# luokn/ms-gat

Measured on AMD Instinct MI355X. Metric: MS-GAT fwd+bwd samples/sec (B×T node-updates/s), PEMSD7 N=883 T=12, higher is better.
Workload: dtype f32

## Files before the change

### ms_gat_amd/csrc/scores.hip

```cpp
#include "common.hpp"

namespace msgat {

constexpr int kRowBlock = 256;

__global__ __launch_bounds__(kBlock) void k_edge_grad(const float* __restrict__ dEp, int nchunks,
                                                      const float* __restrict__ E, const int* __restrict__ epos,
                                                      int stride, float* __restrict__ gE, int nnz) {
  const int g = blockIdx.y;
  const int e = blockIdx.x * kBlock + threadIdx.x;
  if (e >= nnz) return;
  const float* p = dEp + (size_t)g * nchunks * stride + (epos != nullptr ? epos[e] : e);
  float a0 = 0.f, a1 = 0.f, a2 = 0.f, a3 = 0.f;
  int k = 0;
  for (; k + 4 <= nchunks; k += 4) {
    a0 += p[(size_t)(k + 0) * stride];
    a1 += p[(size_t)(k + 1) * stride];
    a2 += p[(size_t)(k + 2) * stride];
    a3 += p[(size_t)(k + 3) * stride];
  }
  for (; k < nchunks; ++k) a0 += p[(size_t)k * stride];
  gE[(size_t)g * nnz + e] = E[(size_t)g * nnz + e] * ((a0 + a1) + (a2 + a3));
}

__global__ __launch_bounds__(kBlock) void k_edge_grad_csc(const float* __restrict__ dEp, int nchunks,
                                                          const float* __restrict__ Ec, const int* __restrict__ cperm,
                                                          float* __restrict__ gE, int nnz) {
  const int g = blockIdx.y;
  const int k = blockIdx.x * kBlock + threadIdx.x;
  if (k >= nnz) return;
  const float* p = dEp + (size_t)g * nchunks * nnz + k;
  float a[8] = {0.f, 0.f, 0.f, 0.f, 0.f, 0.f, 0.f, 0.f};
  const float ec = Ec[(size_t)g * nnz + k];
  const int dst = cperm[k];
  int c = 0;
  for (; c + 8 <= nchunks; c += 8) {
#pragma unroll
    for (int i = 0; i < 8; ++i) a[i] += p[(size_t)(c + i) * nnz];
  }
  for (; c < nchunks; ++c) a[0] += p[(size_t)c * nnz];
  gE[(size_t)g * nnz + dst] = ec * (((a[0] + a[1]) + (a[2] + a[3])) + ((a[4] + a[5]) + (a[6] + a[7])));
}

__global__ __launch_bounds__(kBlock) void k_edge_grad_x(const float* __restrict__ dEp, int nchunks,
                                                        const float* __restrict__ E, const int* __restrict__ epos,
                                                        int stride, float* __restrict__ gE, int nnz,
                                                        const float* __restrict__ dEx) {
  const int g = blockIdx.y;
  const int e = blockIdx.x * kBlock + threadIdx.x;
  if (e >= nnz) return;
  const float* p = dEp + (size_t)g * nchunks * stride + (epos != nullptr ? epos[e] : e);
  float a0 = 0.f, a1 = 0.f, a2 = 0.f, a3 = 0.f;
  int k = 0;
  for (; k + 4 <= nchunks; k += 4) {
    a0 += p[(size_t)(k + 0) * stride];
    a1 += p[(size_t)(k + 1) * stride];
    a2 += p[(size_t)(k + 2) * stride];
    a3 += p[(size_t)(k + 3) * stride];
  }
  for (; k < nchunks; ++k) a0 += p[(size_t)k * stride];
  const size_t i = (size_t)g * nnz + e;
  gE[i] = E[i] * (((a0 + a1) + (a2 + a3)) + dEx[i]);
}

__global__ __launch_bounds__(kBlock) void k_edge_grad_csc_x(const float* __restrict__ dEp, int nchunks,
                                                            const float* __restrict__ Ec, const int* __restrict__ cperm,
                                                            float* __restrict__ gE, int nnz, const float* __restrict__ dEx) {
  const int g = blockIdx.y;
  const int k = blockIdx.x * kBlock + threadIdx.x;
  if (k >= nnz) return;
  const float* p = dEp + (size_t)g * nchunks * nnz + k;
  float a[8] = {0.f, 0.f, 0.f, 0.f, 0.f, 0.f, 0.f, 0.f};
  const float ec = Ec[(size_t)g * nnz + k];
  const int dst = cperm[k];
  int c = 0;
  for (; c + 8 <= nchunks; c += 8) {
#pragma unroll
    for (int i = 0; i < 8; ++i) a[i] += p[(size_t)(c + i) * nnz];
  }
  for (; c < nchunks; ++c) a[0] += p[(size_t)c * nnz];
  const size_t i = (size_t)g * nnz + dst;
  gE[i] = ec * ((((a[0] + a[1]) + (a[2] + a[3])) + ((a[4] + a[5]) + (a[6] + a[7]))) + dEx[i]);
}


template <int T, int DC>
__global__ __launch_bounds__(kRowBlock) void k_bwd_rows(
    const int* __restrict__ rowptr, const int* __restrict__ col, const float* __restrict__ E,
    const float* __restrict__ u, const float* __restrict__ dv,
    const float* __restrict__ q, const float* __restrict__ pq, const float* __restrict__ Wg,
    float* gE, float* __restrict__ delta, float* __restrict__ dkW, float* __restrict__ dq,
    float* __restrict__ dwg_part, int Bg, int N, int nnz, int nblk) {
  constexpr int T4 = T / 4;
  constexpr int DCa = DC < 0 ? -DC : DC;
  constexpr int DCn = DCa > 0 ? DCa : 1;
  __shared__ float qs[kRowBlock * T];
  __shared__ float ds[kRowBlock * T];
  const int g = blockIdx.y;
  const int r = g / Bg;
  const int n = blockIdx.x * kRowBlock + threadIdx.x;
  const bool valid = n < N;
  const int nc = valid ? n : 0;
  const float* qg = q + (size_t)g * N * T;
  float d = 0.f;
  float dk[T], pr[T];
#pragma unroll
  for (int t4 = 0; t4 < T4; ++t4) {
    const float4 v = reinterpret_cast<const float4*>(pq + ((size_t)g * N + nc) * T)[t4];
    pr[4 * t4 + 0] = v.x; pr[4 * t4 + 1] = v.y; pr[4 * t4 + 2] = v.z; pr[4 * t4 + 3] = v.w;
    dk[4 * t4 + 0] = 0.f; dk[4 * t4 + 1] = 0.f; dk[4 * t4 + 2] = 0.f; dk[4 * t4 + 3] = 0.f;
  }
  float4 dvr[DCn][T4];
  if (DCa > 0) {
#pragma unroll
    for (int c = 0; c < DCn; ++c)
#pragma unroll
      for (int t4 = 0; t4 < T4; ++t4)
        dvr[c][t4] = reinterpret_cast<const float4*>(dv + (((size_t)g * DCa + c) * N + nc) * T)[t4];
  }
  auto edge_grad = [&](int e, int ce) -> float {
    float dE;
    if (DCa > 0) {
      dE = 0.f;
#pragma unroll
      for (int c = 0; c < DCn; ++c) {
        const float4* um = reinterpret_cast<const float4*>(u + (((size_t)g * DCa + c) * N + ce) * T);
#pragma unroll
        for (int t4 = 0; t4 < T4; ++t4) dE = f4dot(dvr[c][t4], um[t4], dE);
      }
    } else {
      return gE[(size_t)g * nnz + e];
    }
    if constexpr (DC < 0) dE += gE[(size_t)g * nnz + e];
    return E[(size_t)g * nnz + e] * dE;
  };
  const int e0 = valid ? rowptr[n] : 0;
  const int e1 = valid ? rowptr[n + 1] : 0;
  for (int e = e0; e < e1; e += 4) {
    int ee[4], cc[4];
#pragma unroll
    for (int i = 0; i < 4; ++i) {
      ee[i] = min(e + i, e1 - 1);
      cc[i] = col[ee[i]];
    }
    float gg[4];
#pragma unroll
    for (int i = 0; i < 4; ++i) {
      const float raw = edge_grad(ee[i], cc[i]);
      gg[i] = (e + i < e1) ? raw : 0.f;
    }
    if (DCa > 0) {
#pragma unroll
      for (int i = 0; i < 4; ++i)
        if (e + i < e1) gE[(size_t)g * nnz + ee[i]] = gg[i];
    }
    float4 qv[4][T4];
#pragma unroll
    for (int i = 0; i < 4; ++i)
#pragma unroll
      for (int t4 = 0; t4 < T4; ++t4) qv[i][t4] = reinterpret_cast<const float4*>(qg + (size_t)cc[i] * T)[t4];
#pragma unroll
    for (int i = 0; i < 4; ++i) {
      d += gg[i];
#pragma unroll
      for (int t4 = 0; t4 < T4; ++t4) {
        dk[4 * t4 + 0] = fmaf(gg[i], qv[i][t4].x - pr[4 * t4 + 0], dk[4 * t4 + 0]);
        dk[4 * t4 + 1] = fmaf(gg[i], qv[i][t4].y - pr[4 * t4 + 1], dk[4 * t4 + 1]);
        dk[4 * t4 + 2] = fmaf(gg[i], qv[i][t4].z - pr[4 * t4 + 2], dk[4 * t4 + 2]);
        dk[4 * t4 + 3] = fmaf(gg[i], qv[i][t4].w - pr[4 * t4 + 3], dk[4 * t4 + 3]);
      }
    }
  }
  if (valid) {
    float4* dkdst = reinterpret_cast<float4*>(dkW + ((size_t)g * N + n) * T);
#pragma unroll
    for (int t4 = 0; t4 < T4; ++t4) dkdst[t4] = make_float4(dk[4 * t4], dk[4 * t4 + 1], dk[4 * t4 + 2], dk[4 * t4 + 3]);
    delta[(size_t)g * N + n] = d;
    const float* wg = Wg + (size_t)r * T * T;
    float out[T];
#pragma unroll
    for (int t = 0; t < T; ++t) {
      float a = 0.f;
#pragma unroll
      for (int s = 0; s < T; ++s) a = fmaf(dk[s], wg[t * T + s], a);
      out[t] = a;
    }
    float4* dqdst = reinterpret_cast<float4*>(dq + ((size_t)g * N + n) * T);
#pragma unroll
    for (int t4 = 0; t4 < T4; ++t4) dqdst[t4] = make_float4(out[4 * t4], out[4 * t4 + 1], out[4 * t4 + 2], out[4 * t4 + 3]);
  }
#pragma unroll
  for (int t4 = 0; t4 < T4; ++t4) {
    const float4 v = reinterpret_cast<const float4*>(qg + (size_t)nc * T)[t4];
    reinterpret_cast<float4*>(qs + threadIdx.x * T)[t4] = v;
    reinterpret_cast<float4*>(ds + threadIdx.x * T)[t4] = make_float4(dk[4 * t4], dk[4 * t4 + 1], dk[4 * t4 + 2], dk[4 * t4 + 3]);
  }
  __syncthreads();
  {
    const int wave = threadIdx.x >> 6, lane = threadIdx.x & 63;
    const int i = lane & 15, kq = lane >> 4;
    const int ic = i < T ? i : 0;
    const float keep = i < T ? 1.f : 0.f;
    f32x4 d = {0.f, 0.f, 0.f, 0.f};
#pragma unroll
    for (int k = 0; k < 16; ++k) {
      const int row = 64 * wave + 4 * k + kq;
      d = mfma_16x16x4(qs[row * T + ic] * keep, ds[row * T + ic] * keep, d);
    }
    __syncthreads();
    static_assert(kRowBlock == 256 && kRowBlock * 4 >= 4 * 256, "four waves, one 16x16 tile each");
#pragma unroll
    for (int reg = 0; reg < 4; ++reg) qs[wave * 256 + reg * 64 + lane] = d[reg];
    __syncthreads();
    const int e = threadIdx.x;
    const int t = 4 * ((e & 63) >> 4) + (e >> 6);
    const int sc = e & 15;
    const float v = (qs[e] + qs[256 + e]) + (qs[512 + e] + qs[768 + e]);
    if (t < T && sc < T) dwg_part[((size_t)g * nblk + blockIdx.x) * (T * T) + t * T + sc] = v;
  }
}

size_t dwg_partial_floats(int G, int N, int T) { return (size_t)G * cdiv(N, kRowBlock) * T * T; }
int bwd_rows_direct_max_channels() { return 4; }

int launch_bwd_rows(const msgat_graph_t& gr, const float* dEp, int nchunks, const float* Ecsc, int direct_c,
                    const float* u, const float* dv, const float* E, const float* q, const float* pq, const float* Wg,
                    float* gE, float* delta, float* dkW, float* dq, float* dwg_part, float* dWg, int G, int Bg, int N,
                    int T, hipStream_t s, ReduceJobs* defer, const float* dEx) {
  const int nblk = cdiv(N, kRowBlock);
  dim3 grid(nblk, G);
  const bool partials_in_csc = Ecsc != nullptr;
  if (direct_c == 0 && gr.nnz > 0) {
    dim3 ge(cdiv(gr.nnz, kBlock), G);
    if (partials_in_csc) {
      if (dEx != nullptr)
        hipLaunchKernelGGL(k_edge_grad_csc_x, ge, dim3(kBlock), 0, s, dEp, nchunks, Ecsc, gr.cperm, gE, gr.nnz, dEx);
      else
        hipLaunchKernelGGL(k_edge_grad_csc, ge, dim3(kBlock), 0, s, dEp, nchunks, Ecsc, gr.cperm, gE, gr.nnz);
    } else {
      const bool sell = sell_usable(gr.sell_rows, gr.nnz, N, T);
      if (dEx != nullptr)
        hipLaunchKernelGGL(k_edge_grad_x, ge, dim3(kBlock), 0, s, dEp, nchunks, E, sell ? gr.sell_rows.pos : nullptr,
                           sell ? gr.sell_rows.n_pos : gr.nnz, gE, gr.nnz, dEx);
      else
        hipLaunchKernelGGL(k_edge_grad, ge, dim3(kBlock), 0, s, dEp, nchunks, E, sell ? gr.sell_rows.pos : nullptr,
                           sell ? gr.sell_rows.n_pos : gr.nnz, gE, gr.nnz);
    }
    MSGAT_CHECK_LAUNCH();
  }
  if (direct_c > 0 && dEx != nullptr && gr.nnz > 0) {
    const hipError_t e = hipMemcpyAsync(gE, dEx, sizeof(float) * (size_t)G * gr.nnz, hipMemcpyDeviceToDevice, s);
    if (e != hipSuccess) return MSGAT_ERR_HIP_BASE - (int)e;
  }
#define MSGAT_ROWS(TT, DC)                                                                                          \
  hipLaunchKernelGGL((k_bwd_rows<TT, DC>), grid, dim3(kRowBlock), 0, s, gr.rowptr, gr.col, E, u, dv, q, pq, Wg, gE,  \
                     delta, dkW, dq, dwg_part, Bg, N, gr.nnz, nblk)
#define MSGAT_ROWS_DC(TT, DC)  \
  if (dEx != nullptr)          \
    MSGAT_ROWS(TT, -DC);       \
  else                         \
    MSGAT_ROWS(TT, DC)
#define MSGAT_ROWS_T(TT)                        \
  switch (direct_c) {                           \
    case 0: MSGAT_ROWS(TT, 0); break;           \
    case 1: MSGAT_ROWS_DC(TT, 1); break;        \
    case 2: MSGAT_ROWS_DC(TT, 2); break;        \
    case 3: MSGAT_ROWS_DC(TT, 3); break;        \
    case 4: MSGAT_ROWS_DC(TT, 4); break;        \
    default: return MSGAT_ERR_UNSUPPORTED;      \
  }
  switch (T) {
    case 4: MSGAT_ROWS_T(4); break;
    case 8: MSGAT_ROWS_T(8); break;
    case 12: MSGAT_ROWS_T(12); break;
    case 16: MSGAT_ROWS_T(16); break;
    default: return MSGAT_ERR_UNSUPPORTED;
  }
#undef MSGAT_ROWS_T
#undef MSGAT_ROWS_DC
#undef MSGAT_ROWS
  MSGAT_CHECK_LAUNCH();
  return launch_reduce_groups_defer(dwg_part, G / Bg, Bg * nblk, T * T, dWg, s, defer);
}

}
```

Baseline: 47240.

## Split backward row kernel across T/4 lanes per row with LDS edge staging

Rewrites the backward row kernel so each graph row is handled by T/4 threads, one float4 of the time dimension each, instead of one thread per row. Edge columns and coefficients for the block's row range are staged through shared memory in chunks. Per-edge dot products are reduced across lanes through shared memory. The dq = dk·Wg product moves onto MFMA tiles using the spare waves. The aim is more parallelism, coalesced q gathers and fewer registers per thread, at the cost of extra syncthreads, more LDS use and more complex edge-chunk bookkeeping.

```diff
diff --git a/ms_gat_amd/csrc/scores.hip b/ms_gat_amd/csrc/scores.hip
--- a/ms_gat_amd/csrc/scores.hip
+++ b/ms_gat_amd/csrc/scores.hip
@@ -3,6 +3,7 @@
 namespace msgat {
 
 constexpr int kRowBlock = 256;
+constexpr int kEdgeStage = 1024;
 
 __global__ __launch_bounds__(kBlock) void k_edge_grad(const float* __restrict__ dEp, int nchunks,
                                                       const float* __restrict__ E, const int* __restrict__ epos,
@@ -84,140 +85,198 @@
 }
 
 
+constexpr int bwd_rows_min_waves(int T, int DC) { return (T == 16 || DC > 1 || DC < -1) ? T / 4 : T / 2; }
+
 template <int T, int DC>
-__global__ __launch_bounds__(kRowBlock) void k_bwd_rows(
+__global__ __launch_bounds__(kRowBlock * (T / 4), bwd_rows_min_waves(T, DC)) void k_bwd_rows(
     const int* __restrict__ rowptr, const int* __restrict__ col, const float* __restrict__ E,
     const float* __restrict__ u, const float* __restrict__ dv,
     const float* __restrict__ q, const float* __restrict__ pq, const float* __restrict__ Wg,
     float* gE, float* __restrict__ delta, float* __restrict__ dkW, float* __restrict__ dq,
     float* __restrict__ dwg_part, int Bg, int N, int nnz, int nblk) {
   constexpr int T4 = T / 4;
+  constexpr int NT = kRowBlock * T4;
+  constexpr int NW = NT / 64;
   constexpr int DCa = DC < 0 ? -DC : DC;
   constexpr int DCn = DCa > 0 ? DCa : 1;
-  __shared__ float qs[kRowBlock * T];
-  __shared__ float ds[kRowBlock * T];
+  constexpr int K = (T4 == 4 || DC != 0) ? 4 : 8;
+  constexpr int KU = K / DCn;
+  constexpr int SI = (kEdgeStage + NT - 1) / NT;
+  static_assert(T % 4 == 0 && KU >= 1 && kRowBlock == 256, "four waves' worth of rows, float4 per lane");
+  __shared__ __align__(16) float qs[kRowBlock * T];
+  __shared__ __align__(16) float ds[kRowBlock * T];
+  __shared__ int s_col[kEdgeStage];
+  __shared__ float s_coef[kEdgeStage];
+  __shared__ float s_part[DCa > 0 ? T4 * kEdgeStage : 1];
+  __shared__ float s_gx[DC < 0 ? kEdgeStage : 1];
+  const int tid = threadIdx.x;
   const int g = blockIdx.y;
   const int r = g / Bg;
-  const int n = blockIdx.x * kRowBlock + threadIdx.x;
+  const int rl = tid / T4, j = tid - rl * T4;
+  const int n0 = blockIdx.x * kRowBlock;
+  const int n = n0 + rl;
   const bool valid = n < N;
-  const int nc = valid ? n : 0;
+  const int nc = valid ? n : N - 1;
+  const int wave = tid >> 6, lane = tid & 63;
+  const int mi = lane & 15, kq = lane >> 4;
+  const int mic = mi < T ? mi : 0;
   const float* qg = q + (size_t)g * N * T;
+  const size_t eg = (size_t)g * nnz;
+  const int ebeg = rowptr[n0];
+  const int eend = rowptr[min(n0 + kRowBlock, N)];
+  int e0 = rowptr[nc], e1 = rowptr[nc + 1];
+  if (!valid) e0 = e1 = 0;
+  const float4 pr = *reinterpret_cast<const float4*>(pq + ((size_t)g * N + nc) * T + 4 * j);
+  const float4 qown = *reinterpret_cast<const float4*>(qg + (size_t)nc * T + 4 * j);
+  float4 dvr[DCn];
+  if constexpr (DCa > 0) {
+#pragma unroll
+    for (int c = 0; c < DCn; ++c)
+      dvr[c] = *reinterpret_cast<const float4*>(dv + (((size_t)g * DCa + c) * N + nc) * T + 4 * j);
+  }
+  float wgb[T4];
+#pragma unroll
+  for (int ks = 0; ks < T4; ++ks) {
+    const float w = Wg[(size_t)r * T * T + mic * T + 4 * ks + kq];
+    wgb[ks] = mi < T ? w : 0.f;
+  }
   float d = 0.f;
-  float dk[T], pr[T];
-#pragma unroll
-  for (int t4 = 0; t4 < T4; ++t4) {
-    const float4 v = reinterpret_cast<const float4*>(pq + ((size_t)g * N + nc) * T)[t4];
-    pr[4 * t4 + 0] = v.x; pr[4 * t4 + 1] = v.y; pr[4 * t4 + 2] = v.z; pr[4 * t4 + 3] = v.w;
-    dk[4 * t4 + 0] = 0.f; dk[4 * t4 + 1] = 0.f; dk[4 * t4 + 2] = 0.f; dk[4 * t4 + 3] = 0.f;
-  }
-  float4 dvr[DCn][T4];
-  if (DCa > 0) {
-#pragma unroll
-    for (int c = 0; c < DCn; ++c)
-#pragma unroll
-      for (int t4 = 0; t4 < T4; ++t4)
-        dvr[c][t4] = reinterpret_cast<const float4*>(dv + (((size_t)g * DCa + c) * N + nc) * T)[t4];
-  }
-  auto edge_grad = [&](int e, int ce) -> float {
-    float dE;
-    if (DCa > 0) {
-      dE = 0.f;
-#pragma unroll
-      for (int c = 0; c < DCn; ++c) {
-        const float4* um = reinterpret_cast<const float4*>(u + (((size_t)g * DCa + c) * N + ce) * T);
-#pragma unroll
-        for (int t4 = 0; t4 < T4; ++t4) dE = f4dot(dvr[c][t4], um[t4], dE);
-      }
-    } else {
-      return gE[(size_t)g * nnz + e];
-    }
-    if constexpr (DC < 0) dE += gE[(size_t)g * nnz + e];
-    return E[(size_t)g * nnz + e] * dE;
-  };
-  const int e0 = valid ? rowptr[n] : 0;
-  const int e1 = valid ? rowptr[n + 1] : 0;
-  for (int e = e0; e < e1; e += 4) {
-    int ee[4], cc[4];
-#pragma unroll
-    for (int i = 0; i < 4; ++i) {
-      ee[i] = min(e + i, e1 - 1);
-      cc[i] = col[ee[i]];
-    }
-    float gg[4];
-#pragma unroll
-    for (int i = 0; i < 4; ++i) {
-      const float raw = edge_grad(ee[i], cc[i]);
-      gg[i] = (e + i < e1) ? raw : 0.f;
-    }
-    if (DCa > 0) {
-#pragma unroll
-      for (int i = 0; i < 4; ++i)
-        if (e + i < e1) gE[(size_t)g * nnz + ee[i]] = gg[i];
-    }
-    float4 qv[4][T4];
-#pragma unroll
-    for (int i = 0; i < 4; ++i)
-#pragma unroll
-      for (int t4 = 0; t4 < T4; ++t4) qv[i][t4] = reinterpret_cast<const float4*>(qg + (size_t)cc[i] * T)[t4];
-#pragma unroll
-    for (int i = 0; i < 4; ++i) {
-      d += gg[i];
-#pragma unroll
-      for (int t4 = 0; t4 < T4; ++t4) {
-        dk[4 * t4 + 0] = fmaf(gg[i], qv[i][t4].x - pr[4 * t4 + 0], dk[4 * t4 + 0]);
-        dk[4 * t4 + 1] = fmaf(gg[i], qv[i][t4].y - pr[4 * t4 + 1], dk[4 * t4 + 1]);
-        dk[4 * t4 + 2] = fmaf(gg[i], qv[i][t4].z - pr[4 * t4 + 2], dk[4 * t4 + 2]);
-        dk[4 * t4 + 3] = fmaf(gg[i], qv[i][t4].w - pr[4 * t4 + 3], dk[4 * t4 + 3]);
-      }
-    }
+  float4 dk = f4zero();
+  for (int c0 = ebeg; c0 < eend; c0 += kEdgeStage) {
+    const int cn = min(kEdgeStage, eend - c0);
+    {
+      int cv[SI];
+      float ev[SI], xv[SI];
+#pragma unroll
+      for (int s = 0; s < SI; ++s) {
+        const size_t e = (size_t)c0 + min(tid + s * NT, cn - 1);
+        cv[s] = col[e];
+        ev[s] = DC == 0 ? gE[eg + e] : E[eg + e];
+        xv[s] = DC < 0 ? gE[eg + e] : 0.f;
+      }
+#pragma unroll
+      for (int s = 0; s < SI; ++s) {
+        const int i = tid + s * NT;
+        if (i < cn) {
+          s_col[i] = cv[s];
+          s_coef[i] = ev[s];
+          if constexpr (DC < 0) s_gx[i] = xv[s];
+        }
+      }
+    }
+    __syncthreads();
+    const int lo = max(e0, c0) - c0, hi = min(e1, c0 + cn) - c0;
+    auto slot = [&](int el) { return max(min(el, hi - 1), 0); };
+    float4 qv[K];
+    auto load_q = [&](int el) {
+#pragma unroll
+      for (int i = 0; i < K; ++i)
+        qv[i] = *reinterpret_cast<const float4*>(qg + (size_t)s_col[slot(el + i)] * T + 4 * j);
+    };
+    if constexpr (DCa > 0) {
+      load_q(lo);
+#pragma clang loop unroll(disable) vectorize(disable) interleave(disable)
+      for (int el = lo; el < hi; el += KU) {
+        float4 uv[KU][DCn];
+#pragma unroll
+        for (int i = 0; i < KU; ++i) {
+          const int ce = s_col[slot(el + i)];
+#pragma unroll
+          for (int c = 0; c < DCn; ++c)
+            uv[i][c] = *reinterpret_cast<const float4*>(u + (((size_t)g * DCa + c) * N + ce) * T + 4 * j);
+        }
+#pragma unroll
+        for (int i = 0; i < KU; ++i) {
+          float p = 0.f;
+#pragma unroll
+          for (int c = 0; c < DCn; ++c) p = f4dot(dvr[c], uv[i][c], p);
+          if (el + i < hi) s_part[j * kEdgeStage + el + i] = p;
+        }
+      }
+      __syncthreads();
+#pragma unroll
+      for (int s = 0; s < SI; ++s) {
+        const int i = tid + s * NT;
+        if (i < cn) {
+          float dE = s_part[i];
+#pragma unroll
+          for (int jj = 1; jj < T4; ++jj) dE += s_part[jj * kEdgeStage + i];
+          if constexpr (DC < 0) dE += s_gx[i];
+          const float ge = s_coef[i] * dE;
+          s_coef[i] = ge;
+          gE[eg + c0 + i] = ge;
+        }
+      }
+      __syncthreads();
+    }
+#pragma clang loop unroll(disable) vectorize(disable) interleave(disable)
+    for (int el = lo; el < hi; el += K) {
+      if (DCa == 0 || el > lo) load_q(el);
+      float gg[K];
+#pragma unroll
+      for (int i = 0; i < K; ++i) gg[i] = (el + i < hi) ? s_coef[slot(el + i)] : 0.f;
+#pragma unroll
+      for (int i = 0; i < K; ++i) {
+        d += gg[i];
+        dk.x = fmaf(gg[i], qv[i].x - pr.x, dk.x);
+        dk.y = fmaf(gg[i], qv[i].y - pr.y, dk.y);
+        dk.z = fmaf(gg[i], qv[i].z - pr.z, dk.z);
+        dk.w = fmaf(gg[i], qv[i].w - pr.w, dk.w);
+      }
+    }
+    if (c0 + kEdgeStage < eend) __syncthreads();
   }
   if (valid) {
-    float4* dkdst = reinterpret_cast<float4*>(dkW + ((size_t)g * N + n) * T);
-#pragma unroll
-    for (int t4 = 0; t4 < T4; ++t4) dkdst[t4] = make_float4(dk[4 * t4], dk[4 * t4 + 1], dk[4 * t4 + 2], dk[4 * t4 + 3]);
-    delta[(size_t)g * N + n] = d;
-    const float* wg = Wg + (size_t)r * T * T;
-    float out[T];
-#pragma unroll
-    for (int t = 0; t < T; ++t) {
-      float a = 0.f;
-#pragma unroll
-      for (int s = 0; s < T; ++s) a = fmaf(dk[s], wg[t * T + s], a);
-      out[t] = a;
-    }
-    float4* dqdst = reinterpret_cast<float4*>(dq + ((size_t)g * N + n) * T);
-#pragma unroll
-    for (int t4 = 0; t4 < T4; ++t4) dqdst[t4] = make_float4(out[4 * t4], out[4 * t4 + 1], out[4 * t4 + 2], out[4 * t4 + 3]);
-  }
-#pragma unroll
-  for (int t4 = 0; t4 < T4; ++t4) {
-    const float4 v = reinterpret_cast<const float4*>(qg + (size_t)nc * T)[t4];
-    reinterpret_cast<float4*>(qs + threadIdx.x * T)[t4] = v;
-    reinterpret_cast<float4*>(ds + threadIdx.x * T)[t4] = make_float4(dk[4 * t4], dk[4 * t4 + 1], dk[4 * t4 + 2], dk[4 * t4 + 3]);
-  }
+    *reinterpret_cast<float4*>(dkW + ((size_t)g * N + n) * T + 4 * j) = dk;
+    if (j == 0) delta[(size_t)g * N + n] = d;
+  }
+  reinterpret_cast<float4*>(qs)[tid] = qown;
+  reinterpret_cast<float4*>(ds)[tid] = dk;
   __syncthreads();
-  {
-    const int wave = threadIdx.x >> 6, lane = threadIdx.x & 63;
-    const int i = lane & 15, kq = lane >> 4;
-    const int ic = i < T ? i : 0;
-    const float keep = i < T ? 1.f : 0.f;
-    f32x4 d = {0.f, 0.f, 0.f, 0.f};
+  f32x4 dw = f32x4_zero();
+  if (wave < 4) {
+    const float keep = mi < T ? 1.f : 0.f;
 #pragma unroll
     for (int k = 0; k < 16; ++k) {
       const int row = 64 * wave + 4 * k + kq;
-      d = mfma_16x16x4(qs[row * T + ic] * keep, ds[row * T + ic] * keep, d);
-    }
-    __syncthreads();
-    static_assert(kRowBlock == 256 && kRowBlock * 4 >= 4 * 256, "four waves, one 16x16 tile each");
-#pragma unroll
-    for (int reg = 0; reg < 4; ++reg) qs[wave * 256 + reg * 64 + lane] = d[reg];
-    __syncthreads();
-    const int e = threadIdx.x;
+      dw = mfma_16x16x4(qs[row * T + mic] * keep, ds[row * T + mic] * keep, dw);
+    }
+  }
+  constexpr int QW = NW > 4 ? NW - 4 : NW;
+  constexpr int QT = (16 + QW - 1) / QW;
+  const int qw = NW > 4 ? wave - 4 : wave;
+  f32x4 dqt[QT];
+#pragma unroll
+  for (int s = 0; s < QT; ++s) {
+    dqt[s] = f32x4_zero();
+    const int tile = qw + s * QW;
+    if (qw >= 0 && tile < 16) {
+#pragma unroll
+      for (int ks = 0; ks < T4; ++ks) dqt[s] = mfma_16x16x4(ds[(16 * tile + mi) * T + 4 * ks + kq], wgb[ks], dqt[s]);
+    }
+  }
+  __syncthreads();
+  if (wave < 4) {
+#pragma unroll
+    for (int reg = 0; reg < 4; ++reg) qs[wave * 256 + reg * 64 + lane] = dw[reg];
+  }
+#pragma unroll
+  for (int s = 0; s < QT; ++s) {
+    const int tile = qw + s * QW;
+    if (qw >= 0 && tile < 16 && mi < T) {
+#pragma unroll
+      for (int reg = 0; reg < 4; ++reg) ds[(16 * tile + 4 * kq + reg) * T + mi] = dqt[s][reg];
+    }
+  }
+  __syncthreads();
+  if (tid < 256) {
+    const int e = tid;
     const int t = 4 * ((e & 63) >> 4) + (e >> 6);
     const int sc = e & 15;
     const float v = (qs[e] + qs[256 + e]) + (qs[512 + e] + qs[768 + e]);
     if (t < T && sc < T) dwg_part[((size_t)g * nblk + blockIdx.x) * (T * T) + t * T + sc] = v;
   }
+  if (valid) *reinterpret_cast<float4*>(dq + ((size_t)g * N + n) * T + 4 * j) = reinterpret_cast<const float4*>(ds)[tid];
 }
 
 size_t dwg_partial_floats(int G, int N, int T) { return (size_t)G * cdiv(N, kRowBlock) * T * T; }
@@ -253,8 +312,8 @@
     if (e != hipSuccess) return MSGAT_ERR_HIP_BASE - (int)e;
   }
 #define MSGAT_ROWS(TT, DC)                                                                                          \
-  hipLaunchKernelGGL((k_bwd_rows<TT, DC>), grid, dim3(kRowBlock), 0, s, gr.rowptr, gr.col, E, u, dv, q, pq, Wg, gE,  \
-                     delta, dkW, dq, dwg_part, Bg, N, gr.nnz, nblk)
+  hipLaunchKernelGGL((k_bwd_rows<TT, DC>), grid, dim3(kRowBlock * (TT / 4)), 0, s, gr.rowptr, gr.col, E, u, dv, q, pq,  \
+                     Wg, gE, delta, dkW, dq, dwg_part, Bg, N, gr.nnz, nblk)
 #define MSGAT_ROWS_DC(TT, DC)  \
   if (dEx != nullptr)          \
     MSGAT_ROWS(TT, -DC);       \
```

Result: no change. 47400 (median of 6 runs) (+0.3%).
